# daigo0927/tf-raft

Measured on NVIDIA H100. Metric: frame-pairs/sec at 448×512 iters=12; final-flow max-abs vs ref, higher is better.
Workload: dtype f32

## Files before the change

include/raft_b200.h:

```cpp
#ifndef RAFT_B200_H_
#define RAFT_B200_H_

#include <stddef.h>
#include <stdint.h>

#ifdef __cplusplus
extern "C" {
#endif

#define RAFT_B200_ABI_VERSION 2
#define RAFT_MAX_LEVELS 8

typedef enum raft_status {
  RAFT_OK = 0,
  RAFT_ERR_BAD_ARG = -1,
  RAFT_ERR_BAD_SHAPE = -2,
  RAFT_ERR_WORKSPACE = -3,
  RAFT_ERR_NO_DEVICE = -4,
  RAFT_ERR_DRIVER = -5,
  RAFT_ERR_UNSUPPORTED = -6
} raft_status;

typedef enum raft_precision { RAFT_PREC_FP32 = 0, RAFT_PREC_F16X2 = 1 } raft_precision;

// ... 90 lines not shown
  RAFT_METRIC_LT1 = 1,
  RAFT_METRIC_LT3 = 2,
  RAFT_METRIC_LT5 = 3,
  RAFT_METRIC_OUTLIER = 4,
  RAFT_METRIC_COUNTS = 5
};

int raft_b200_flow_metrics_workspace_bytes(int B, int H, int W, size_t* bytes);

int raft_b200_flow_metrics(const float* pred, const float* gt, const float* valid, int B, int H, int W, int use_max_flow,
                           float max_flow, void* workspace, size_t workspace_bytes, long long* counts, double* sums,
                           void* stream);


typedef struct raft_conv {
  const float* kernel;
  const float* bias;
  int kh, kw, cin, cout;
} raft_conv;

typedef struct raft_basic_weights {
  raft_conv convc1, convc2, convf1, convf2, conv;
  raft_conv convz1, convr1, convq1, convz2, convr2, convq2;
  raft_conv fh_conv1, fh_conv2;
  raft_conv mask0, mask2;
} raft_basic_weights;

typedef struct raft_small_weights {
  raft_conv convc1, convf1, convf2, conv;
  raft_conv convz, convr, convq;
  raft_conv fh_conv1, fh_conv2;
} raft_small_weights;

int raft_b200_update_prepared_bytes(int variant, int corr_channels, int precision, size_t* bytes);
int raft_b200_update_prepare(int variant, const void* weights ,
                             void* prepared, size_t prepared_bytes, int precision, void* stream);

int raft_b200_update_workspace_bytes(int variant, int B, int h, int w, int precision, size_t* bytes);

int raft_b200_update_basic(const void* prepared, const float* net, const float* inp, const float* corr,
                           const float* flow, float* net_out, float* mask_or_null, float* delta_flow, int B,
                           int h, int w, void* workspace, size_t workspace_bytes, int precision, void* stream);

int raft_b200_update_small(const void* prepared, const float* net, const float* inp, const float* corr,
                           const float* flow, float* net_out, float* delta_flow, int B, int h, int w,
                           void* workspace, size_t workspace_bytes, int precision, void* stream);


typedef struct raft_norm {
  const float* gamma;
  const float* beta;
  const float* moving_mean;
  const float* moving_variance;
} raft_norm;

typedef struct raft_resblock {
  raft_conv conv1, conv2;
  raft_norm norm1, norm2;
  raft_conv downsample;
  raft_norm downsample_norm;
} raft_resblock;

typedef struct raft_encoder_weights {
  raft_conv conv1;
  raft_norm norm1;
  raft_resblock block[6];
  raft_conv conv2;
} raft_encoder_weights;

typedef enum raft_norm_type { RAFT_NORM_NONE = 0, RAFT_NORM_INSTANCE = 1, RAFT_NORM_BATCH = 2 } raft_norm_type;

int raft_b200_encoder_prepared_bytes(int variant, int out_dim, size_t* bytes);
int raft_b200_encoder_prepare(int variant, int norm_type, int out_dim, const raft_encoder_weights* weights,
                              void* prepared, size_t prepared_bytes, void* stream);
int raft_b200_encoder_workspace_bytes(int variant, int N, int H, int W, size_t* bytes);

int raft_b200_encoder_forward(int variant, int norm_type, int out_dim, const void* prepared, const float* images,
                              int N, int H, int W, int training, int image_norm, float* out, void* workspace,
                              size_t workspace_bytes, void* stream);

int raft_b200_context_split(const float* cnet, int npix, int hidden, int context, float* net, float* inp,
                            void* stream);

int raft_b200_conv2d(const float* x, const float* kernel, const float* bias, int B, int H, int W, int cin, int kh,
                     int kw, int cout, int act, float* out, int out_stride, int out_c0, void* stream);


int raft_b200_upsample_convex(const float* flow, const float* mask, int B, int h, int w, float* out, void* stream);

int raft_b200_upflow8(const float* flow, int B, int h, int w, float* out, void* stream);

int raft_b200_forward_loop(int variant, const void* prepared, const float* const pyr[], int levels, int radius,
                           float* net, const float* inp, float* coords1, float* const flow_up[], int iters,
                           int B, int h, int w, void* workspace, size_t workspace_bytes, int precision,
                           void* stream);

long long raft_b200_launch_count(void);
void raft_b200_launch_count_reset(void);
void raft_b200_profile_loop(int enable);
int raft_b200_profile_read(float* lookup_ms, float* update_ms, int* iterations);

#ifdef __cplusplus
}
#endif
#endif
```

tf_raft_b200/_lib.py:

```python
import ctypes
import os

import torch

_HERE = os.path.dirname(os.path.abspath(__file__))
LIB_PATH = os.environ.get('RAFT_B200_LIB') or os.path.join(_HERE, 'libraft_b200.so')

PREC_FP32 = 0
PREC_F16X2 = 1
VARIANT_BASIC = 0
VARIANT_SMALL = 1
MAX_LEVELS = 8

_PRECISIONS = {'fp32': PREC_FP32, 'f16x2': PREC_F16X2, PREC_FP32: PREC_FP32, PREC_F16X2: PREC_F16X2}


def resolve_precision(precision=None):
    if precision is None:
        precision = os.environ.get('RAFT_B200_PRECISION', 'f16x2')
    try:
        return _PRECISIONS[precision]
    except KeyError:
        raise ValueError(f'unknown precision {precision!r}; expected one of fp32, f16x2') from None


class RaftConv(ctypes.Structure):
    _fields_ = [('kernel', ctypes.c_void_p), ('bias', ctypes.c_void_p),
                ('kh', ctypes.c_int), ('kw', ctypes.c_int), ('cin', ctypes.c_int), ('cout', ctypes.c_int)]


class RaftNorm(ctypes.Structure):
    _fields_ = [('gamma', ctypes.c_void_p), ('beta', ctypes.c_void_p), ('moving_mean', ctypes.c_void_p),
                ('moving_variance', ctypes.c_void_p)]


class RaftResBlock(ctypes.Structure):
    _fields_ = [('conv1', RaftConv), ('conv2', RaftConv), ('norm1', RaftNorm), ('norm2', RaftNorm),
                ('downsample', RaftConv), ('downsample_norm', RaftNorm)]


class RaftEncoderWeights(ctypes.Structure):
    _fields_ = [('conv1', RaftConv), ('norm1', RaftNorm), ('block', RaftResBlock * 6), ('conv2', RaftConv)]


NORM_TYPES = {None: 0, 'instance': 1, 'batch': 2}

_vp, _i, _sz = ctypes.c_void_p, ctypes.c_int, ctypes.c_size_t
_SIGNATURES = {
    'raft_b200_strerror': (ctypes.c_char_p, [_i]),
    'raft_b200_abi_version': (_i, []),
    'raft_b200_device_ok': (_i, [_i]),
    'raft_b200_launch_count': (ctypes.c_longlong, []),
    'raft_b200_launch_count_reset': (None, []),
    'raft_b200_profile_loop': (None, [_i]),
    'raft_b200_profile_read': (_i, [ctypes.POINTER(ctypes.c_float), ctypes.POINTER(ctypes.c_float), ctypes.POINTER(_i)]),
    'raft_b200_corr_pyramid_sizes': (_i, [_i, _i, _i, _i, ctypes.POINTER(_sz)]),
    'raft_b200_corr_workspace_bytes': (_i, [_i, _i, _i, _i, _i, _i, ctypes.POINTER(_sz)]),
    'raft_b200_corr_pyramid_build': (_i, [_vp, _vp, _i, _i, _i, _i, _i, ctypes.POINTER(_vp), _vp, _sz, _i, _vp]),
    'raft_b200_corr_lookup': (_i, [ctypes.POINTER(_vp), _vp, _i, _i, _i, _i, _i, _vp, _i, _vp]),
    'raft_b200_corr_lookup_backward': (_i, [ctypes.POINTER(_vp), _vp, _vp, _i, _i, _i, _i, _i, _vp, ctypes.POINTER(_vp), _vp]),
    'raft_b200_sumsq': (_i, [_vp, _sz, _vp, _sz, _vp, _vp]),
    'raft_b200_adamw_step': (_i, [_vp, _vp, _vp, _vp, _sz, _vp, ctypes.c_float, ctypes.c_float, ctypes.c_float,
                                  ctypes.c_float, ctypes.c_float, ctypes.c_float, _vp]),
    'raft_b200_bilinear_sampler': (_i, [_vp, _vp, _i, _i, _i, _i, _vp, _vp]),
    'raft_b200_coords_grid': (_i, [_i, _i, _i, _vp, _vp]),
    'raft_b200_forward_interpolate': (_i, [_vp, _i, _i, _i, _vp, _vp]),
    'raft_b200_coords_init': (_i, [_vp, _i, _i, _i, _vp, _vp]),
    'raft_b200_fb_occlusion': (_i, [_vp, _vp, _i, _i, _i, ctypes.c_float, ctypes.c_float, _vp, _vp, _vp]),
    'raft_b200_augment_workspace_bytes': (_i, [_vp, _i, _i, ctypes.POINTER(_sz)]),
    'raft_b200_augment_dense': (_i, [_vp, _vp, _i, _vp, _sz, _vp]),
    'raft_b200_augment_sparse': (_i, [_vp, _vp, _i, _vp, _sz, _vp]),
    'raft_b200_flow_to_image': (_i, [_vp, _vp, _i, _i, _i, _i, _i, ctypes.c_float, _i, _vp, _i, _vp, _vp, _vp, _vp]),
    'raft_b200_png16_flow_decode': (_i, [_vp, _sz, _vp, _vp, _i, _vp, _vp]),
    'raft_b200_flow_metrics_workspace_bytes': (_i, [_i, _i, _i, ctypes.POINTER(_sz)]),
    'raft_b200_flow_metrics': (_i, [_vp, _vp, _vp, _i, _i, _i, _i, ctypes.c_float, _vp, _sz, _vp, _vp, _vp]),
    'raft_b200_update_prepared_bytes':(_i, [_i, _i, _i, ctypes.POINTER(_sz)]),
    'raft_b200_update_prepare': (_i, [_i, _vp, _vp, _sz, _i, _vp]),
    'raft_b200_update_workspace_bytes': (_i, [_i, _i, _i, _i, _i, ctypes.POINTER(_sz)]),
    'raft_b200_update_basic': (_i, [_vp, _vp, _vp, _vp, _vp, _vp, _vp, _vp, _i, _i, _i, _vp, _sz, _i, _vp]),
    'raft_b200_update_small': (_i, [_vp, _vp, _vp, _vp, _vp, _vp, _vp, _i, _i, _i, _vp, _sz, _i, _vp]),
    'raft_b200_upsample_convex': (_i, [_vp, _vp, _i, _i, _i, _vp, _vp]),
    'raft_b200_upflow8': (_i, [_vp, _i, _i, _i, _vp, _vp]),
    'raft_b200_encoder_prepared_bytes': (_i, [_i, _i, ctypes.POINTER(_sz)]),
    'raft_b200_encoder_prepare': (_i, [_i, _i, _i, _vp, _vp, _sz, _vp]),
    'raft_b200_encoder_workspace_bytes': (_i, [_i, _i, _i, _i, ctypes.POINTER(_sz)]),
    'raft_b200_encoder_forward': (_i, [_i, _i, _i, _vp, _vp, _i, _i, _i, _i, _i, _vp, _vp, _sz, _vp]),
    'raft_b200_context_split': (_i, [_vp, _i, _i, _i, _vp, _vp, _vp]),
    'raft_b200_conv2d': (_i, [_vp, _vp, _vp, _i, _i, _i, _i, _i, _i, _i, _i, _vp, _i, _i, _vp]),
    'raft_b200_forward_loop': (_i, [_i, _vp, ctypes.POINTER(_vp), _i, _i, _vp, _vp, _vp, ctypes.POINTER(_vp), _i,
                                    _i, _i, _i, _vp, _sz, _i, _vp]),
}
EXPORTED_SYMBOLS = tuple(_SIGNATURES)

_lib = None


def lib():
    global _lib
    if _lib is None:
        if not os.path.exists(LIB_PATH):
            raise ImportError(
                f'{LIB_PATH} is missing: the sm_90a CUDA library has not been built. '
                'Run `python -c "import __graft_entry__ as g; g.build()"` (or `python -m tf_raft_b200.build`) '
                'from the repository root. There is no CPU / PyTorch fallback for the RAFT hot path.')
        handle = ctypes.CDLL(LIB_PATH)
        for name, (res, args) in _SIGNATURES.items():
            fn = getattr(handle, name)
            fn.restype = res
            fn.argtypes = args
        if handle.raft_b200_abi_version() != 2:
            raise ImportError('libraft_b200.so ABI version mismatch; rebuild it')
        _lib = handle
    return _lib


def strerror(status):
    return lib().raft_b200_strerror(status).decode()


def check(status, what=''):
    if status != 0:
        raise RuntimeError(f'raft_b200 {what} failed: [{status}] {strerror(status)}')


def ptr(t):
    return ctypes.c_void_p(None if t is None else t.data_ptr())


def ptr_array(tensors):
    return (ctypes.c_void_p * len(tensors))(*[None if t is None else t.data_ptr() for t in tensors])


def stream():
    return ctypes.c_void_p(torch.cuda.current_stream().cuda_stream)


def require_cuda(*tensors):
    for t in tensors:
        if t is None:
            continue
        if not t.is_cuda:
            raise RuntimeError('tf_raft_b200 runs on CUDA tensors only (sm_90a); got a CPU tensor. '
                               'There is no CPU fallback for this path.')
        if t.dtype != torch.float32 or not t.is_contiguous():
            raise RuntimeError('expected contiguous float32 tensors')


def f32c(t):
    if not t.is_cuda:
        raise RuntimeError('tf_raft_b200 runs on CUDA tensors only (sm_90a); got a CPU tensor. '
                           'There is no CPU fallback for this path.')
    return t.to(torch.float32).contiguous()


def workspace(nbytes, device):
    return torch.empty(max(int(nbytes), 16), dtype=torch.uint8, device=device)


def launch_count():
    return int(lib().raft_b200_launch_count())


def launch_count_reset():
    lib().raft_b200_launch_count_reset()
```

tf_raft_b200/csrc/api.cu:

```cuda
#include <float.h>
#include <limits.h>
#include <stdlib.h>

#include <algorithm>

#include "augment.cuh"
#include "corr_tc.cuh"
#include "dataset.cuh"
#include "encoder.cuh"
#include "flow_viz.cuh"
#include "train.cuh"
#include "video.cuh"

namespace raft {
thread_local long long g_launches = 0;

static int check_dims(int B, int h, int w) { return (B > 0 && h > 0 && w > 0) ? 0 : RAFT_ERR_BAD_SHAPE; }
static int check_variant(int v) { return (v == RAFT_VARIANT_BASIC || v == RAFT_VARIANT_SMALL) ? 0 : RAFT_ERR_BAD_ARG; }
static int check_precision(int p) { return (p == RAFT_PREC_FP32 || p == RAFT_PREC_F16X2) ? 0 : RAFT_ERR_BAD_ARG; }

struct LoopProfile {
  bool on = false;
  int n = 0;
  cudaEvent_t ev[64][3];
// ... 31 lines not shown
  W.total = off;
  return W;
}

static int corr_build_fp32(const float* f1, const float* f2, int B, int h, int w, int C, int levels, float* const pyr[],
                           cudaStream_t st) {
  const int N = h * w;
  dim3 grid((unsigned)ceil_div(N, 64), (unsigned)ceil_div(N, 64), (unsigned)B);
  RAFT_TRY(launch(corr_fp32_kernel, grid, 256, 0, st, f1, f2, pyr[0], N, C, sqrtf((float)C)));
  int lh = h, lw = w;
  for (int l = 1; l < levels; ++l) {
    const size_t M = (size_t)B * N;
    const size_t total = M * (lh / 2) * (lw / 2);
    RAFT_TRY(launch(avgpool2x2_kernel, grid_for(total), 256, 0, st, pyr[l - 1], pyr[l], M, lh, lw, 1));
    lh /= 2;
    lw /= 2;
  }
  return 0;
}

static int corr_build_tc(const float* f1, const float* f2, int B, int h, int w, int C, int levels, float* const pyr[],
                         void* ws, cudaStream_t st) {
  if (C % kChunkK != 0) return RAFT_ERR_BAD_SHAPE;
  CorrWs W = corr_ws_layout(ws, B, h, w, C, levels, RAFT_PREC_F16X2);
  const int N = h * w;
  const size_t npix = (size_t)B * N;
  if (levels <= 4) {
    CorrPrepParams q;
    memset(&q, 0, sizeof(q));
    q.f1 = f1; q.f2 = f2; q.f1_hi = W.f1_hi; q.f1_lo = W.f1_lo;
    for (int l = 0; l < levels; ++l) { q.f2_hi[l] = W.f2_hi[l]; q.f2_lo[l] = W.f2_lo[l]; }
    q.B = B; q.h = h; q.w = w; q.C = C; q.levels = levels;
    q.patches_x = ceil_div(w, 8); q.patches_y = ceil_div(h, 8);
    q.npatch = B * q.patches_x * q.patches_y;
    const int split_blocks = (int)std::min<size_t>((npix * C / 4 + 127) / 128, (size_t)kNumSMs * 8);
    RAFT_TRY(launch(corr_prep_kernel, q.npatch + split_blocks, 128, 0, st, q));
  } else {
    RAFT_TRY(launch(split_plane_kernel, grid_for(npix * C), 256, 0, st, f1, C, 0, C, C, W.f1_hi, W.f1_lo, C, 0, npix, 1.0f));
    int lh = h, lw = w;
    const float* src = f2;
    for (int l = 0; l < levels; ++l) {
      if (l > 0) {
        const size_t total = (size_t)B * (lh / 2) * (lw / 2) * C;
        RAFT_TRY(launch(avgpool2x2_kernel, grid_for(total), 256, 0, st, src, W.f2_lvl[l], (size_t)B, lh, lw, C));
        src = W.f2_lvl[l];
        lh /= 2;
        lw /= 2;
      }
      const size_t np2 = (size_t)B * lh * lw;
      RAFT_TRY(launch(split_plane_kernel, grid_for(np2 * C), 256, 0, st, src, C, 0, C, C, W.f2_hi[l], W.f2_lo[l], C, 0, np2,
                      1.0f));
    }
  }

  CorrTcParams p;
  memset(&p, 0, sizeof(p));
  RAFT_TRY(make_tmap_act2(&p.a_map, W.f1_hi, W.f1_lo, B, 1, N, C, 128, 1));
  p.levels = levels; p.B = B; p.N = N; p.chunks = C / kChunkK;
  p.mtiles_img = ceil_div(N, kTileM);
  const int mtiles = B * p.mtiles_img;
  int lh = h, lw = w;
  for (int l = 0; l < levels; ++l) {
    const int N2 = lh * lw;
    const int ntn = ceil_div(N2, kCorrBn);
    const int bn = round_up(ceil_div(N2, ntn), 16);
    RAFT_TRY(make_tmap_wgt2(&p.b_map[l], W.f2_hi[l], W.f2_lo[l], B, N2, C, bn));
    p.out[l] = pyr[l];
    p.n2[l] = N2; p.bn[l] = bn;
    p.tile0[l + 1] = p.tile0[l] + mtiles * ntn;
    lh /= 2;
    lw /= 2;
  }
  p.corr_div = sqrtf((float)C);
  {
    int e = 0;
    const float m = frexpf(p.corr_div, &e);
    p.corr_mul = (m == 0.5f && p.corr_div * p.corr_div == (float)C) ? 1.0f / p.corr_div : 0.0f;
  }
  unsigned grid = 0;
  RAFT_TRY(persistent_grid<corr_tc_kernel>(kCorrSmemBytes, p.tile0[levels], &grid));
  return launch(corr_tc_kernel, grid, kTcThreads, kCorrSmemBytes, st, p);
}

static int update_begin(const UpdateCtx& c, const float* h, const float* inp) {
  const Workspace& W = c.W;
  const VariantDims d = variant_dims(c.variant);
  const size_t npix = (size_t)c.B * c.h * c.w;
  if (c.precision == RAFT_PREC_F16X2) {
    RAFT_CUDA_TRY(cudaMemsetAsync(W.f16_begin, 0, W.f16_bytes, c.stream));
    RAFT_TRY(launch(split_plane_kernel, grid_for(npix * d.ctx), 256, 0, c.stream, inp, d.ctx, 0, d.ctx, d.ctx, W.x_hi, W.x_lo,
                    d.s_x, 0, npix, 1.0f));
    return launch(split_plane_kernel, grid_for(npix * d.hid), 256, 0, c.stream, h, d.hid, 0, d.hid, d.hid, W.h_hi, W.h_lo,
                  d.s_h, 0, npix, 1.0f);
  }
  RAFT_CUDA_TRY(cudaMemsetAsync(W.x, 0, npix * d.c_x * sizeof(float), c.stream));
  return launch(copy_channels_kernel, grid_for(npix * d.ctx), 256, 0, c.stream, inp, d.ctx, 0, W.x, d.c_x, 0, d.ctx, npix);
}

static int make_ctx(UpdateCtx& c, int variant, const void* prepared, int B, int h, int w, void* ws, size_t ws_bytes,
                    int precision, void* stream) {
  RAFT_TRY(check_variant(variant));
  RAFT_TRY(check_precision(precision));
  if (!prepared || !ws) return RAFT_ERR_BAD_ARG;
  RAFT_TRY(check_dims(B, h, w));
  c.variant = variant; c.precision = precision; c.B = B; c.h = h; c.w = w;
  c.prepared = reinterpret_cast<const uint8_t*>(prepared);
  c.PL = prepared_layout(variant, precision);
  c.W = workspace_layout(ws, variant, B, h, w, precision);
  if (c.W.total > ws_bytes) return RAFT_ERR_WORKSPACE;
  c.stream = reinterpret_cast<cudaStream_t>(stream);
  c.plan = nullptr;
  c.fim_ready = false;
  return 0;
}

static bool mega_enabled() {
  static const int v = [] { const char* e = getenv("RAFT_B200_MEGA"); return e ? atoi(e) : 1; }();
  return v != 0;
}
static int update_block_tc(UpdateCtx& c, float* h, float* delta, float* mask, float* adv_coords) {
  MegaPlan plan;
  c.plan = mega_enabled() ? &plan : nullptr;
  const int st = update_core_tc(c, h, delta, mask, adv_coords);
  c.plan = nullptr;
  RAFT_TRY(st);
  if (!mega_enabled()) return 0;
  return mega_launch(plan, c.W.mega_flags, c.W.mega_flag_words, true, c.stream);
}

static int update_once(int variant, const void* prepared, const float* net, const float* inp, const float* corr,
                       const float* flow, float* net_out, float* mask, float* delta, int B, int h, int w, void* ws,
                       size_t ws_bytes, int precision, void* stream) {
  if (!net || !inp || !corr || !flow || !net_out || !delta) return RAFT_ERR_BAD_ARG;
  UpdateCtx c;
  RAFT_TRY(make_ctx(c, variant, prepared, B, h, w, ws, ws_bytes, precision, stream));
  const VariantDims d = variant_dims(variant);
  const size_t npix = (size_t)B * h * w;
  if (net_out != net)
    RAFT_CUDA_TRY(cudaMemcpyAsync(net_out, net, npix * d.hid * sizeof(float), cudaMemcpyDeviceToDevice, c.stream));
  RAFT_CUDA_TRY(cudaMemcpyAsync(c.W.flow, flow, npix * 2 * sizeof(float), cudaMemcpyDeviceToDevice, c.stream));
  RAFT_TRY(update_begin(c, net_out, inp));
  if (precision == RAFT_PREC_F16X2) {
    RAFT_TRY(launch(split_plane_kernel, grid_for(npix * d.s_corr), 256, 0, c.stream, corr, d.corr_ch, 0, d.corr_ch, d.s_corr,
                    c.W.corr_hi, c.W.corr_lo, d.s_corr, 0, npix, 1.0f));
    return update_block_tc(c, net_out, delta, mask, nullptr);
  }
  RAFT_CUDA_TRY(cudaMemcpyAsync(c.W.corr, corr, npix * d.corr_ch * sizeof(float), cudaMemcpyDeviceToDevice, c.stream));
  return update_core_fp32(c, net_out, delta, mask);
}

static int lookup_launch(const float* const pyr[], const float* coords, int B, int h, int w, int levels, int radius,
                         float* out, int out_stride, __half* out_hi, __half* out_lo, int h_stride, int h_pad,
                         cudaStream_t st, const float* im_flow = nullptr, __half* im_hi = nullptr, __half* im_lo = nullptr) {
  LookupParams p;
  memset(&p, 0, sizeof(p));
  int lh = h, lw = w;
  for (int l = 0; l < levels; ++l) {
    if (lh < 1 || lw < 1) return RAFT_ERR_BAD_SHAPE;
    p.pyr[l] = pyr[l];
    p.lh[l] = lh;
    p.lw[l] = lw;
    lh /= 2;
    lw /= 2;
  }
  p.coords = coords;
  p.out = out; p.out_stride = out_stride;
// ... 371 lines not shown
int raft_b200_update_workspace_bytes(int variant, int B, int h, int w, int precision, size_t* bytes) {
  if (!bytes) return RAFT_ERR_BAD_ARG;
  RAFT_TRY(check_variant(variant));
  RAFT_TRY(check_precision(precision));
  RAFT_TRY(check_dims(B, h, w));
  *bytes = workspace_layout(nullptr, variant, B, h, w, precision).total;
  return RAFT_OK;
}

int raft_b200_update_basic(const void* prepared, const float* net, const float* inp, const float* corr,
                           const float* flow, float* net_out, float* mask_or_null, float* delta_flow, int B, int h,
                           int w, void* workspace, size_t workspace_bytes, int precision, void* stream) {
  return update_once(RAFT_VARIANT_BASIC, prepared, net, inp, corr, flow, net_out, mask_or_null, delta_flow, B, h, w,
                     workspace, workspace_bytes, precision, stream);
}

int raft_b200_update_small(const void* prepared, const float* net, const float* inp, const float* corr,
                           const float* flow, float* net_out, float* delta_flow, int B, int h, int w, void* workspace,
                           size_t workspace_bytes, int precision, void* stream) {
  return update_once(RAFT_VARIANT_SMALL, prepared, net, inp, corr, flow, net_out, nullptr, delta_flow, B, h, w,
                     workspace, workspace_bytes, precision, stream);
}

int raft_b200_upsample_convex(const float* flow, const float* mask, int B, int h, int w, float* out, void* stream) {
  if (!flow || !mask || !out) return RAFT_ERR_BAD_ARG;
  RAFT_TRY(check_dims(B, h, w));
  const size_t npix = (size_t)B * h * w;
  return launch(upsample_convex_kernel, grid_for(npix, 4, kNumSMs * 32), 256, 0, reinterpret_cast<cudaStream_t>(stream), flow,
                mask, B, h, w, out);
}

int raft_b200_upflow8(const float* flow, int B, int h, int w, float* out, void* stream) {
  if (!flow || !out) return RAFT_ERR_BAD_ARG;
  RAFT_TRY(check_dims(B, h, w));
  return launch(upflow8_kernel, grid_for((size_t)B * h * w * 64), 256, 0, reinterpret_cast<cudaStream_t>(stream), flow, B, h,
                w, out);
}

int raft_b200_encoder_prepared_bytes(int variant, int out_dim, size_t* bytes) {
  if (!bytes) return RAFT_ERR_BAD_ARG;
  RAFT_TRY(check_variant(variant));
  if (out_dim < 32 || out_dim > 256 || out_dim % 32) return RAFT_ERR_BAD_SHAPE;
  *bytes = enc_layout(variant, out_dim).total;
  return RAFT_OK;
}

int raft_b200_encoder_prepare(int variant, int norm_type, int out_dim, const raft_encoder_weights* weights,
                              void* prepared, size_t prepared_bytes, void* stream) {
  if (!weights || !prepared) return RAFT_ERR_BAD_ARG;
  RAFT_TRY(check_variant(variant));
  if (norm_type < 0 || norm_type > 2) return RAFT_ERR_BAD_ARG;
  if (out_dim < 32 || out_dim > 256 || out_dim % 32) return RAFT_ERR_BAD_SHAPE;
  return encoder_prepare(variant, norm_type, out_dim, weights, prepared, prepared_bytes, reinterpret_cast<cudaStream_t>(stream));
}

int raft_b200_encoder_workspace_bytes(int variant, int N, int H, int W, size_t* bytes) {
  if (!bytes) return RAFT_ERR_BAD_ARG;
  RAFT_TRY(check_variant(variant));
  RAFT_TRY(check_dims(N, H, W));
  *bytes = enc_ws_layout(nullptr, variant, N, H, W).total;
  return RAFT_OK;
}

int raft_b200_encoder_forward(int variant, int norm_type, int out_dim, const void* prepared, const float* images,
                              int N, int H, int W, int training, int image_norm, float* out, void* workspace,
                              size_t workspace_bytes, void* stream) {
  if (!prepared || !images || !out || !workspace) return RAFT_ERR_BAD_ARG;
  RAFT_TRY(check_variant(variant));
  if (norm_type < 0 || norm_type > 2) return RAFT_ERR_BAD_ARG;
  RAFT_TRY(check_dims(N, H, W));
  if (out_dim < 32 || out_dim > 256 || out_dim % 32 || H < 8 || W < 8) return RAFT_ERR_BAD_SHAPE;
  return encoder_forward(variant, norm_type, out_dim, prepared, images, N, H, W, training, image_norm, out, workspace, workspace_bytes,
                         reinterpret_cast<cudaStream_t>(stream));
}

int raft_b200_context_split(const float* cnet, int npix, int hidden, int context, float* net, float* inp,
                            void* stream) {
  if (!cnet || !net || !inp) return RAFT_ERR_BAD_ARG;
  if (npix < 1 || hidden < 1 || context < 1) return RAFT_ERR_BAD_SHAPE;
  return launch(context_split_kernel, grid_for((size_t)npix * (hidden + context)), 256, 0, reinterpret_cast<cudaStream_t>(stream),
                cnet, (size_t)npix, hidden, context, net, inp);
}

int raft_b200_conv2d(const float* x, const float* kernel, const float* bias, int B, int H, int W, int cin, int kh,
                     int kw, int cout, int act, float* out, int out_stride, int out_c0, void* stream) {
  if (!x || !kernel || !out) return RAFT_ERR_BAD_ARG;
  RAFT_TRY(check_dims(B, H, W));
  if (cin < 1 || cout < 1 || kh < 1 || kw < 1 || !(kh & 1) || !(kw & 1) || act < 0 || act > 3) return RAFT_ERR_BAD_SHAPE;
  if (out_stride < out_c0 + cout) return RAFT_ERR_BAD_SHAPE;
  SimtConvParams p;
  memset(&p, 0, sizeof(p));
  p.src[0] = x; p.src_stride[0] = cin; p.src_c0[0] = 0; p.src_n[0] = cin; p.nsrc = 1;
  p.w = kernel; p.bias = bias;
  p.kh = kh; p.kw = kw; p.cin = cin; p.cout = cout;
  p.B = B; p.H = H; p.W = W;
  p.out = out; p.out_stride = out_stride; p.out_c0 = out_c0;
  p.act = act; p.out_scale = 1.0f;
  dim3 grid((unsigned)ceil_div(B * H * W, 64), (unsigned)ceil_div(cout, 64));
  return launch(conv_simt_kernel, grid, 256, 0, reinterpret_cast<cudaStream_t>(stream), p);
}

int raft_b200_forward_loop(int variant, const void* prepared, const float* const pyr[], int levels, int radius,
                           float* net, const float* inp, float* coords1, float* const flow_up[], int iters, int B,
                           int h, int w, void* workspace, size_t workspace_bytes, int precision, void* stream) {
  if (!pyr || !net || !inp || !coords1 || !flow_up || iters < 0) return RAFT_ERR_BAD_ARG;
  if (levels < 1 || levels > RAFT_MAX_LEVELS || radius < 0) return RAFT_ERR_BAD_ARG;
  UpdateCtx c;
  RAFT_TRY(make_ctx(c, variant, prepared, B, h, w, workspace, workspace_bytes, precision, stream));
  const VariantDims d = variant_dims(variant);
  const int side = 2 * radius + 1;
  if (levels * side * side != d.corr_ch) return RAFT_ERR_BAD_SHAPE;
  const size_t npix = (size_t)B * h * w;
  const Workspace& W = c.W;
  RAFT_TRY(update_begin(c, net, inp));
  RAFT_TRY(launch(flow_advance_kernel, grid_for(npix), 256, 0, c.stream, coords1, nullptr, W.flow, B, h, w));
  const bool prof = g_prof.on && iters <= 64;
  if (prof && !g_prof.created) {
    for (int i = 0; i < 64; ++i)
      for (int k = 0; k < 3; ++k) RAFT_CUDA_TRY(cudaEventCreate(&g_prof.ev[i][k]));
    g_prof.created = true;
  }
  if (prof) g_prof.n = iters;
  for (int i = 0; i < iters; ++i) {
    float* mask = (variant == RAFT_VARIANT_BASIC && flow_up[i]) ? W.mask : nullptr;
    if (precision == RAFT_PREC_F16X2) {
      if (prof) RAFT_CUDA_TRY(cudaEventRecord(g_prof.ev[i][0], c.stream));
      RAFT_TRY(lookup_launch(pyr, coords1, B, h, w, levels, radius, nullptr, 0, W.corr_hi, W.corr_lo, d.s_corr, d.s_corr,
                             c.stream, W.flow, W.fim_hi, W.fim_lo));
      if (prof) RAFT_CUDA_TRY(cudaEventRecord(g_prof.ev[i][1], c.stream));
      c.fim_ready = true;
      RAFT_TRY(update_block_tc(c, net, W.delta, mask, coords1));
      c.fim_ready = false;
      if (prof) RAFT_CUDA_TRY(cudaEventRecord(g_prof.ev[i][2], c.stream));
    } else {
      RAFT_TRY(lookup_launch(pyr, coords1, B, h, w, levels, radius, W.corr, d.corr_ch, nullptr, nullptr, 0, 0, c.stream));
      RAFT_TRY(update_core_fp32(c, net, W.delta, mask));
      RAFT_TRY(launch(flow_advance_kernel, grid_for(npix), 256, 0, c.stream, coords1, W.delta, W.flow, B, h, w));
    }
    if (flow_up[i]) {
      if (variant == RAFT_VARIANT_BASIC)
        RAFT_TRY(raft_b200_upsample_convex(W.flow, W.mask, B, h, w, flow_up[i], stream));
      else
        RAFT_TRY(raft_b200_upflow8(W.flow, B, h, w, flow_up[i], stream));
    }
  }
  return raft_launch_status();
}

}
```

tf_raft_b200/csrc/encoder.cuh:

```cuda
#pragma once
#include <algorithm>

#include "lookup.cuh"
#include "update.cuh"

namespace raft {

enum { NORM_NONE = 0, NORM_INSTANCE = 1, NORM_BATCH = 2 };

struct EncSpec { int c0; int c[3]; int s[3]; };
inline EncSpec enc_spec(int variant) {
  if (variant == RAFT_VARIANT_BASIC) return {64, {64, 96, 128}, {1, 2, 2}};
  return {32, {32, 64, 96}, {1, 2, 2}};
}
inline int pad64(int c) { return round_up(c, 64); }

struct EncNormSlot { size_t gamma, beta, fscale, fshift; int C; };
struct EncLayout {
  TcWeightSlot conv1;
  EncNormSlot norm1;
  TcWeightSlot bc1[6], bc2[6], bds[6];
  EncNormSlot bn1[6], bn2[6], bnd[6];
  int has_ds[6], bc[6], bstride[6];
  TcWeightSlot conv2;
// ... 99 lines not shown
  const EncLayout L = enc_layout(variant, out_dim);
  if (L.total > bytes) return RAFT_ERR_WORKSPACE;
  const EncSpec S = enc_spec(variant);
  uint8_t* base = reinterpret_cast<uint8_t*>(prepared);
  RAFT_CUDA_TRY(cudaMemsetAsync(base, 0, L.total, st));
  RAFT_TRY(enc_pack_conv(w->conv1, 7, 7, 3, S.c0, L.conv1, true, base, st));
  RAFT_TRY(enc_pack_norm(w->norm1, L.norm1, norm_type, base, st));
  int cin = S.c0;
  for (int k = 0; k < 6; ++k) {
    const int c = L.bc[k];
    RAFT_TRY(enc_pack_conv(w->block[k].conv1, 3, 3, cin, c, L.bc1[k], false, base, st));
    RAFT_TRY(enc_pack_conv(w->block[k].conv2, 3, 3, c, c, L.bc2[k], false, base, st));
    RAFT_TRY(enc_pack_norm(w->block[k].norm1, L.bn1[k], norm_type, base, st));
    RAFT_TRY(enc_pack_norm(w->block[k].norm2, L.bn2[k], norm_type, base, st));
    if (L.has_ds[k]) {
      RAFT_TRY(enc_pack_conv(w->block[k].downsample, 1, 1, cin, c, L.bds[k], false, base, st));
      RAFT_TRY(enc_pack_norm(w->block[k].downsample_norm, L.bnd[k], norm_type, base, st));
    }
    cin = c;
  }
  RAFT_TRY(enc_pack_conv(w->conv2, 1, 1, cin, out_dim, L.conv2, false, base, st));
  return raft_launch_status();
}

struct EncCtx {
  const uint8_t* prep; EncLayout L; EncWs W; cudaStream_t st;
  int N, norm_type, stats;
  int per_image;
};

inline int enc_norm_apply(const EncCtx& c, const EncNormSlot& ns, const float* y, size_t npix, int P, int relu,
                          const float* skip32, const __half* skip_hi, const __half* skip_lo, float* out32, __half* hi,
                          __half* lo) {
  const int C = ns.C, G = c.per_image ? c.N : 1;
  const int Pg = c.per_image ? P : (int)npix;
  const float* gamma = reinterpret_cast<const float*>(c.prep + ns.gamma);
  const float* beta = reinterpret_cast<const float*>(c.prep + ns.beta);
  RAFT_TRY(launch(norm_stats_kernel, dim3((unsigned)G, kNormSplit), 256, 0, c.st, y, Pg, C, kNormSplit, c.W.part));
  RAFT_TRY(launch(norm_final_kernel, ceil_div(G * C * 32, 256), 256, 0, c.st, c.W.part, G, C, kNormSplit, gamma, 1e-3f,
                  c.W.mean, c.W.mult));
  return launch(norm_apply_kernel, grid_for(npix * (pad64(C) / 8)), 256, 0, c.st, y, npix, P, C, c.per_image, c.W.mean,
                c.W.mult, beta, relu, skip32, skip_hi, skip_lo, out32, hi, lo, pad64(C));
}

inline int enc_conv_tc(const EncCtx& c, const TcWeightSlot& cs, int cout, const EncNormSlot* ns, const __half* ahi,
                       const __half* alo, int Hin, int Win, int Hout, int Wout, int stride, int relu, const float* skip,
                       float* out32, __half* ohi, __half* olo) {
  TcConvParams p;
  memset(&p, 0, sizeof(p));
  int tw, th;
  tc_pick_tile(Wout, Hout, &tw, &th);
  if (tw * stride > 256) tw = 128 / stride, th = 128 / tw;
  const int nsplit = tc_n_split(cs.cout_pad);
  if (!nsplit) return RAFT_ERR_BAD_SHAPE;
  RAFT_TRY(make_tmap_act2(&p.a_map[0], ahi, alo, c.N, Hin, Win, cs.cin_pad, tw, th, stride));
  RAFT_TRY(tc_use_weights(p, c.prep, cs, cs.cout_pad / nsplit));
  p.nseg = 1; p.seg_chunks[0] = cs.cin_pad / kChunkK; p.seg_c0[0] = 0;
  p.stride = stride;
  if (stride == 1) { p.ph = (cs.kh - 1) / 2; p.pw = (cs.kw - 1) / 2; }
  else {
    const int tot_h = (Hout - 1) * stride + cs.kh - Hin, tot_w = (Wout - 1) * stride + cs.kw - Win;
    p.ph = (tot_h > 0 ? tot_h : 0) / 2; p.pw = (tot_w > 0 ? tot_w : 0) / 2;
  }
  p.B = c.N; p.H = Hout; p.W = Wout; p.TH = th; p.TW = tw;
  p.n_total = cout;
  p.mode = EPI_LINEAR; p.out_scale = 1.0f;
  p.out_f32 = out32; p.f32_stride = cout; p.f32_c0 = 0;
  p.out_hi = ohi; p.out_lo = olo; p.h_stride = pad64(cout); p.h_c0 = 0;
  if (ns && !c.stats && c.norm_type == NORM_BATCH) {
    p.post_scale = reinterpret_cast<const float*>(c.prep + ns->fscale);
    p.post_shift = reinterpret_cast<const float*>(c.prep + ns->fshift);
  }
  const bool fused = !(ns && c.stats);
  if (fused) {
    p.act = relu ? ACT_RELU : ACT_NONE;
    p.residual = skip; p.res_stride = cout; p.res_c0 = 0;
  } else {
    p.act = ACT_NONE; p.out_hi = nullptr; p.out_lo = nullptr;
  }
  p.group_chunks = 5;
  return tc_launch(p, nsplit, c.st);
}

inline int encoder_forward(int variant, int norm_type, int out_dim, const void* prepared, const float* images, int N,
                           int H, int W, int training, int image_norm, float* out, void* ws, size_t ws_bytes, cudaStream_t st) {
  EncCtx c;
  c.prep = reinterpret_cast<const uint8_t*>(prepared);
  c.L = enc_layout(variant, out_dim);
  c.W = enc_ws_layout(ws, variant, N, H, W);
  if (c.W.total > ws_bytes) return RAFT_ERR_WORKSPACE;
  c.st = st; c.N = N; c.norm_type = norm_type;
  c.stats = (norm_type == NORM_INSTANCE) || (norm_type == NORM_BATCH && training);
  c.per_image = norm_type == NORM_INSTANCE;
  const EncSpec S = enc_spec(variant);
  const EncLayout& L = c.L;
  const EncWs& E = c.W;

  int h = (H + 1) / 2, w = (W + 1) / 2;
  {
    const size_t npix = (size_t)N * h * w;
    const int tot_h = (h - 1) * 2 + 7 - H, tot_w = (w - 1) * 2 + 7 - W;
    const float* src = images;
    if (image_norm) {
      const size_t nimg = (size_t)N * H * W * 3;
      RAFT_TRY(launch(image_norm_kernel, grid_for(nimg), 256, 0, st, images, E.O32, nimg));
      src = E.O32;
    }
    RAFT_TRY(launch(stem_im2col_kernel, grid_for(npix * 24), 256, 0, st, src, N, H, W, h, w, (tot_h > 0 ? tot_h : 0) / 2,
                    (tot_w > 0 ? tot_w : 0) / 2, 0, E.Ih, E.Il));
    if (!c.stats && pad64(S.c0) != S.c0) {
      RAFT_CUDA_TRY(cudaMemsetAsync(E.Xh, 0, npix * pad64(S.c0) * 2, st));
      RAFT_CUDA_TRY(cudaMemsetAsync(E.Xl, 0, npix * pad64(S.c0) * 2, st));
    }
    RAFT_TRY(enc_conv_tc(c, L.conv1, S.c0, &L.norm1, E.Ih, E.Il, h, w, h, w, 1, 1, nullptr, c.stats ? E.Y32 : E.X32, E.Xh, E.Xl));
    if (c.stats) RAFT_TRY(enc_norm_apply(c, L.norm1, E.Y32, npix, h * w, 1, nullptr, nullptr, nullptr, nullptr, E.Xh, E.Xl));
  }

  float *X32 = E.X32, *O32 = E.O32;
  __half *Xh = E.Xh, *Xl = E.Xl, *Oh = E.Oh, *Ol = E.Ol;
  for (int k = 0; k < 6; ++k) {
    const int st2 = L.bstride[k], cc = L.bc[k];
    const int ho = (h + st2 - 1) / st2, wo = (w + st2 - 1) / st2;
    const size_t npo = (size_t)N * ho * wo;
    const bool zero_pad_out = pad64(cc) != cc;
    if (!c.stats && zero_pad_out) {
      RAFT_CUDA_TRY(cudaMemsetAsync(E.Fh, 0, npo * pad64(cc) * 2, st));
      RAFT_CUDA_TRY(cudaMemsetAsync(E.Fl, 0, npo * pad64(cc) * 2, st));
      RAFT_CUDA_TRY(cudaMemsetAsync(Oh, 0, npo * pad64(cc) * 2, st));
      RAFT_CUDA_TRY(cudaMemsetAsync(Ol, 0, npo * pad64(cc) * 2, st));
    }
    RAFT_TRY(enc_conv_tc(c, L.bc1[k], cc, &L.bn1[k], Xh, Xl, h, w, ho, wo, st2, 1, nullptr, c.stats ? E.Y32 : nullptr, E.Fh, E.Fl));
    if (c.stats) RAFT_TRY(enc_norm_apply(c, L.bn1[k], E.Y32, npo, ho * wo, 1, nullptr, nullptr, nullptr, nullptr, E.Fh, E.Fl));
    const float* skip = X32;
    if (L.has_ds[k]) {
      RAFT_TRY(enc_conv_tc(c, L.bds[k], cc, &L.bnd[k], Xh, Xl, h, w, ho, wo, st2, 0, nullptr, c.stats ? E.Y32 : E.D32, nullptr, nullptr));
      if (c.stats) RAFT_TRY(enc_norm_apply(c, L.bnd[k], E.Y32, npo, ho * wo, 0, nullptr, nullptr, nullptr, E.D32, nullptr, nullptr));
      skip = E.D32;
    }
    RAFT_TRY(enc_conv_tc(c, L.bc2[k], cc, &L.bn2[k], E.Fh, E.Fl, ho, wo, ho, wo, 1, 1, skip, c.stats ? E.Y32 : O32, Oh, Ol));
    if (c.stats) {
      if (L.has_ds[k]) RAFT_TRY(enc_norm_apply(c, L.bn2[k], E.Y32, npo, ho * wo, 1, E.D32, nullptr, nullptr, nullptr, Oh, Ol));
      else RAFT_TRY(enc_norm_apply(c, L.bn2[k], E.Y32, npo, ho * wo, 1, nullptr, Xh, Xl, nullptr, Oh, Ol));
    }
    float* t32 = X32; X32 = O32; O32 = t32;
    __half* th_ = Xh; Xh = Oh; Oh = th_;
    __half* tl_ = Xl; Xl = Ol; Ol = tl_;
    h = ho; w = wo;
  }
  RAFT_TRY(enc_conv_tc(c, L.conv2, out_dim, nullptr, Xh, Xl, h, w, h, w, 1, 0, nullptr, out, nullptr, nullptr));
  return raft_launch_status();
}

}
```

tf_raft_b200/model.py:

```python
from collections import OrderedDict

import torch

from . import _lib
from .layers.corr import CorrBlock, coords_grid, coords_init, fb_occlusion, forward_interpolate, upflow8
from .layers.extractor import BasicEncoder, SmallEncoder
from .layers.update import BasicUpdateBlock, SmallUpdateBlock
from .losses import end_point_error, sequence_loss


class RAFT:
    _variant = _lib.VARIANT_BASIC

    def __init__(self, drop_rate=0, iters=12, iters_pred=24, *, precision=None, device='cuda', seed=None,
                 use_graph=False, encoder_backend=None, **kwargs):
        self.hidden_dim = 128
        self.context_dim = 128
        self.corr_levels = 4
        self.corr_radius = 4
        self.drop_rate = drop_rate
        self.iters = iters
        self.iters_pred = iters_pred
        self.precision = _lib.resolve_precision(precision)
        self.device = torch.device(device)
        self.use_graph = use_graph
        self.encoder_backend = encoder_backend
        self._build_layers(seed)
        self._graphs = {}
        self.flow_metrics = None
        self.optimizer = None
        self._trainer = None
        self._params_stale = False

    def _encoder_backend(self):
        return self.encoder_backend or ('native' if self.precision == _lib.PREC_F16X2 else 'torch')

    def _build_layers(self, seed):
        s = 0 if seed is None else seed
        self.fnet = BasicEncoder(output_dim=256, norm_type='instance', drop_rate=self.drop_rate, device=self.device,
                                 seed=s, backend=self._encoder_backend())
        self.cnet = BasicEncoder(output_dim=self.hidden_dim + self.context_dim, norm_type='batch',
                                 drop_rate=self.drop_rate, device=self.device, seed=s + 1, backend=self._encoder_backend())
        self.update_block = BasicUpdateBlock(filters=self.hidden_dim, precision=self.precision, device=self.device,
                                             seed=s + 2)

    def load_params(self, params):
        self.fnet.load_params(params, 'fnet.')
        self.cnet.load_params(params, 'cnet.')
        self.update_block.load_params(params, 'update_block.')
        self._graphs.clear()
        self._trainer = None
        self._params_stale = False

    def state_dict(self):
        self._sync_trained_params()
        out = OrderedDict()
        out.update(self.fnet.state_dict('fnet.'))
        out.update(self.cnet.state_dict('cnet.'))
        out.update(self.update_block.state_dict('update_block.'))
        return out

    def initialize_flow(self, image):
        bs, h, w, _ = image.shape
        return coords_grid(bs, h // 8, w // 8, self.device), coords_grid(bs, h // 8, w // 8, self.device)

    def upsample_flow(self, flow, mask):
        flow, mask = _lib.f32c(flow), _lib.f32c(mask)
        b, h, w, _ = flow.shape
        if tuple(mask.shape) != (b, h, w, 576):
            raise ValueError(f'mask: expected {(b, h, w, 576)}, got {tuple(mask.shape)}')
        out = torch.empty((b, 8 * h, 8 * w, 2), dtype=torch.float32, device=flow.device)
        with torch.cuda.device(flow.device):
            _lib.check(_lib.lib().raft_b200_upsample_convex(_lib.ptr(flow), _lib.ptr(mask), b, h, w, _lib.ptr(out),
                                                            _lib.stream()), 'upsample_convex')
        return out

    def _encode(self, image1, image2, training):
        fmap1, fmap2 = self.fnet([image1, image2], training=training, raw_image=True)
        net, inp = self._context(image1, training)
        return fmap1, fmap2, net, inp

    def _context(self, image1, training):
        cnet = self.cnet(image1, training=training, raw_image=True)
        b, h, w, _ = cnet.shape
        net = torch.empty((b, h, w, self.hidden_dim), dtype=torch.float32, device=cnet.device)
        inp = torch.empty((b, h, w, self.context_dim), dtype=torch.float32, device=cnet.device)
        with torch.cuda.device(cnet.device):
            _lib.check(_lib.lib().raft_b200_context_split(_lib.ptr(cnet), b * h * w, self.hidden_dim,
                                                          self.context_dim, _lib.ptr(net), _lib.ptr(inp),
                                                          _lib.stream()), 'context_split')
        return net, inp

    def _loop(self, corr_block, net, inp, coords1, flow_ups, b, h, w):
        ub = self.update_block
        ws = ub.workspace(b, h, w)
        with torch.cuda.device(self.device):
            _lib.check(_lib.lib().raft_b200_forward_loop(
                self._variant, _lib.ptr(ub.prepared()), _lib.ptr_array(corr_block.corr_pyramid), self.corr_levels,
                self.corr_radius, _lib.ptr(net), _lib.ptr(inp), _lib.ptr(coords1), _lib.ptr_array(flow_ups),
                len(flow_ups), b, h, w, _lib.ptr(ws), ws.numel(), self.precision, _lib.stream()), 'forward_loop')

    def __call__(self, inputs, training, *, last_only=False, flow_init=None):
        image1, image2 = inputs
        image1, image2 = _lib.f32c(image1), _lib.f32c(image2)
        if flow_init is not None:
            flow_init = self._check_flow_init(flow_init, image1)
        self._sync_trained_params()
        if self.use_graph and not training:
            key = (tuple(image1.shape), bool(last_only), flow_init is not None)
            return self._graph_run(key, lambda a, b, f: self._forward(a, b, False, last_only, f),
                                   (image1, image2, flow_init))
        return self._forward(image1, image2, training, last_only, flow_init)

    @staticmethod
    def _check_flow_init(flow_init, image):
        if not isinstance(flow_init, torch.Tensor):
            raise TypeError(f'flow_init must be a torch tensor, got {type(flow_init).__name__}')
        if flow_init.dtype != torch.float32:
            raise TypeError(f'flow_init must be float32, got {flow_init.dtype}')
        if flow_init.device != image.device:
            raise ValueError(f'flow_init is on {flow_init.device}, the images on {image.device}')
        bs, H, W, _ = image.shape
        want = (bs, H // 8, W // 8, 2)
        if tuple(flow_init.shape) != want:
            raise ValueError(f'flow_init: expected {want} for {H}x{W} images, got {tuple(flow_init.shape)}')
        return flow_init.contiguous()

    def _graph_run(self, key, fn, inputs):
        entry = self._graphs.get(key)
        if entry is None:
            statics = [None if t is None else t.clone() for t in inputs]
            side = torch.cuda.Stream(device=self.device)
            side.wait_stream(torch.cuda.current_stream(self.device))
            with torch.cuda.stream(side):
                for _ in range(2):
                    fn(*statics)
            torch.cuda.current_stream(self.device).wait_stream(side)
            torch.cuda.synchronize(self.device)
            graph = torch.cuda.CUDAGraph()
            with torch.cuda.graph(graph):
                outs = fn(*statics)
            keep = [list(m._ws.values()) for m in (self.fnet, self.cnet, self.update_block)]
            entry = (graph, statics, outs, self._last, keep)
            self._graphs[key] = entry
        graph, statics, outs, last, _keep = entry
        for s, t in zip(statics, inputs):
            if t is not None:
                s.copy_(t, non_blocking=True)
        graph.replay()
        self._last = last
        return outs

    @staticmethod
    def _check_size(H, W):
        if H % 8 or W % 8:
            raise ValueError(f'image height and width must be multiples of 8 (got {H}x{W}); the reference fails in '
                             'update.py:146 for other sizes -- crop-or-pad first (datasets/dataset.py:323-334)')

    def _forward(self, image1, image2, training, last_only, flow_init=None):
        bs, H, W, _ = image1.shape
        self._check_size(H, W)
        fmap1, fmap2, net, inp = self._encode(image1, image2, training)
        return self._iterate(fmap1, fmap2, net, inp, bs, H, W, training, last_only, flow_init)

    def _iterate(self, fmap1, fmap2, net, inp, bs, H, W, training, last_only, flow_init):
        h, w = H // 8, W // 8
        iters = self.iters if training else self.iters_pred
        corr_block = CorrBlock(fmap1, fmap2, num_levels=self.corr_levels, radius=self.corr_radius,
                               precision=self.precision)
        if flow_init is None:
            coords1 = coords_grid(bs, h, w, self.device)
        else:
            coords1 = coords_init(flow_init)
        preds = [torch.empty((bs, H, W, 2), dtype=torch.float32, device=self.device)
                 if (not last_only or i == iters - 1) else None for i in range(iters)]
        if iters:
            self._loop(corr_block, net, inp, coords1, preds, bs, h, w)
        self._last = dict(net=net, coords1=coords1, corr_block=corr_block)
        return [p for p in preds if p is not None] if last_only else preds

    def predict_bidirectional(self, inputs):
        image1, image2 = inputs
        image1, image2 = _lib.f32c(image1), _lib.f32c(image2)
        if image1.shape != image2.shape:
            raise ValueError(f'image1 {tuple(image1.shape)} and image2 {tuple(image2.shape)} differ in shape')
        if self.iters_pred < 1:
            raise ValueError('predict_bidirectional needs iters_pred >= 1')
        self._sync_trained_params()
        if self.use_graph:
            return self._graph_run(('bidirectional', tuple(image1.shape)), self._bidirectional, (image1, image2))
        return self._bidirectional(image1, image2)

    def _bidirectional(self, image1, image2):
        bs, H, W, _ = image1.shape
        self._check_size(H, W)
        images = torch.cat([image1, image2])
        fmap = self.fnet(images, training=False, raw_image=True)
        net, inp = self._context(images, False)
        return self._iterate_bidirectional(fmap, torch.cat([fmap[bs:], fmap[:bs]]), net, inp, bs, H, W, None)

    def _iterate_bidirectional(self, fmap1, fmap2, net, inp, bs, H, W, flow_init):
        flow = self._iterate(fmap1, fmap2, net, inp, 2 * bs, H, W, False, True, flow_init)[-1]
        flow_fw, flow_bw = flow[:bs], flow[bs:]
        return (flow_fw, flow_bw) + fb_occlusion(flow_fw, flow_bw)

    def predict_video(self, frames, *, warm_start=True, bidirectional=False):
        self._sync_trained_params()
        if self.iters_pred < 1:
            raise ValueError('predict_video needs iters_pred >= 1')
        shape = coords0 = frame_prev = fmap_prev = flow_init = ctx_prev = None
        for t, frame in enumerate(frames):
            frame = _lib.f32c(frame)
            if shape is None:
                shape = tuple(frame.shape)
                if len(shape) != 4 or shape[-1] != 3:
                    raise ValueError(f'frames must be (B, H, W, 3); got {shape}')
                bs, H, W, _ = shape
                self._check_size(H, W)
            elif tuple(frame.shape) != shape:
                raise ValueError(f'frame {t}: shape {tuple(frame.shape)} differs from the first frame {shape}')
            fmap = self.fnet(frame, training=False, raw_image=True)
            if bidirectional:
                ctx = self._context(frame, False)
            if frame_prev is not None:
                if bidirectional:
# ... 99 lines not shown
```

Before: 311.8.

## Run fnet and cnet encoders concurrently on side streams with shared stem im2col

Adds a fused encode_pair entry point that forks the caller stream into three streams. fnet on image2, fnet on image1 and cnet on image1 then run concurrently, and the image1 stem normalisation and im2col is computed once and shared by both image1 encoders. The goal is to fill the GPU during the small-batch encoder phase and drop one redundant stem pass. In exchange it adds per-device static streams and events, a larger workspace holding three encoder scratch areas, and stream-priority choices that may interact with CUDA graph capture.

```diff
diff --git a/include/raft_b200.h b/include/raft_b200.h
--- a/include/raft_b200.h
+++ b/include/raft_b200.h
@@ -196,6 +196,12 @@
 int raft_b200_context_split(const float* cnet, int npix, int hidden, int context, float* net, float* inp,
                             void* stream);
 
+int raft_b200_encode_pair_workspace_bytes(int variant, int N, int H, int W, int cnet_dim, size_t* bytes);
+int raft_b200_encode_pair(int variant, const void* fnet_prepared, int fnet_norm, int fnet_dim, const void* cnet_prepared,
+                          int cnet_norm, int hidden, int context, const float* image1, const float* image2, int N, int H,
+                          int W, float* fmap1, float* fmap2, float* net, float* inp, void* workspace, size_t workspace_bytes,
+                          void* stream);
+
 int raft_b200_conv2d(const float* x, const float* kernel, const float* bias, int B, int H, int W, int cin, int kh,
                      int kw, int cout, int act, float* out, int out_stride, int out_c0, void* stream);
 
diff --git a/tf_raft_b200/_lib.py b/tf_raft_b200/_lib.py
--- a/tf_raft_b200/_lib.py
+++ b/tf_raft_b200/_lib.py
@@ -86,6 +86,9 @@
     'raft_b200_encoder_workspace_bytes': (_i, [_i, _i, _i, _i, ctypes.POINTER(_sz)]),
     'raft_b200_encoder_forward': (_i, [_i, _i, _i, _vp, _vp, _i, _i, _i, _i, _i, _vp, _vp, _sz, _vp]),
     'raft_b200_context_split': (_i, [_vp, _i, _i, _i, _vp, _vp, _vp]),
+    'raft_b200_encode_pair_workspace_bytes': (_i, [_i, _i, _i, _i, _i, ctypes.POINTER(_sz)]),
+    'raft_b200_encode_pair': (_i, [_i, _vp, _i, _i, _vp, _i, _i, _i, _vp, _vp, _i, _i, _i, _vp, _vp, _vp, _vp, _vp, _sz,
+                                   _vp]),
     'raft_b200_conv2d': (_i, [_vp, _vp, _vp, _i, _i, _i, _i, _i, _i, _i, _i, _vp, _i, _i, _vp]),
     'raft_b200_forward_loop': (_i, [_i, _vp, ctypes.POINTER(_vp), _i, _i, _vp, _vp, _vp, ctypes.POINTER(_vp), _i,
                                     _i, _i, _i, _vp, _sz, _i, _vp]),
diff --git a/tf_raft_b200/csrc/api.cu b/tf_raft_b200/csrc/api.cu
--- a/tf_raft_b200/csrc/api.cu
+++ b/tf_raft_b200/csrc/api.cu
@@ -137,6 +137,49 @@
   return launch(corr_tc_kernel, grid, kTcThreads, kCorrSmemBytes, st, p);
 }
 
+struct PairWs {
+  void* enc[3];
+  size_t enc_bytes;
+  const __half *stem_hi, *stem_lo;
+  float* cnet_out;
+  size_t total;
+};
+static PairWs pair_ws_layout(void* base, int variant, int N, int H, int W, int cnet_dim) {
+  PairWs P;
+  memset(&P, 0, sizeof(P));
+  uint8_t* b8 = reinterpret_cast<uint8_t*>(base);
+  P.enc_bytes = align_up(enc_ws_layout(nullptr, variant, N, H, W).total, 1024);
+  for (int i = 0; i < 3; ++i) P.enc[i] = b8 + i * P.enc_bytes;
+  const EncWs E = enc_ws_layout(P.enc[0], variant, N, H, W);
+  P.stem_hi = E.Ih; P.stem_lo = E.Il;
+  P.cnet_out = reinterpret_cast<float*>(b8 + 3 * P.enc_bytes);
+  P.total = 3 * P.enc_bytes + (size_t)N * ceil_div(H, 8) * ceil_div(W, 8) * cnet_dim * sizeof(float);
+  return P;
+}
+
+struct PairStreams { cudaStream_t s[3]; cudaEvent_t fork, stem, a, b, c; bool ready; };
+static int pair_streams(cudaStream_t caller, PairStreams** out) {
+  static thread_local PairStreams tab[64];
+  int dev = 0;
+  RAFT_CUDA_TRY(cudaGetDevice(&dev));
+  if (dev < 0 || dev >= 64) return RAFT_ERR_UNSUPPORTED;
+  PairStreams& ps = tab[dev];
+  if (!ps.ready) {
+    cudaStreamCaptureStatus cs = cudaStreamCaptureStatusNone;
+    RAFT_CUDA_TRY(cudaStreamIsCapturing(caller, &cs));
+    if (cs != cudaStreamCaptureStatusNone) return RAFT_ERR_UNSUPPORTED;
+    int least = 0, greatest = 0;
+    RAFT_CUDA_TRY(cudaDeviceGetStreamPriorityRange(&least, &greatest));
+    for (int i = 0; i < 3; ++i)
+      RAFT_CUDA_TRY(cudaStreamCreateWithPriority(&ps.s[i], cudaStreamNonBlocking, i < 2 ? greatest : least));
+    for (cudaEvent_t* e : {&ps.fork, &ps.stem, &ps.a, &ps.b, &ps.c})
+      RAFT_CUDA_TRY(cudaEventCreateWithFlags(e, cudaEventDisableTiming));
+    ps.ready = true;
+  }
+  *out = &ps;
+  return RAFT_OK;
+}
+
 static int update_begin(const UpdateCtx& c, const float* h, const float* inp) {
   const Workspace& W = c.W;
   const VariantDims d = variant_dims(c.variant);
@@ -674,6 +717,57 @@
                 cnet, (size_t)npix, hidden, context, net, inp);
 }
 
+int raft_b200_encode_pair_workspace_bytes(int variant, int N, int H, int W, int cnet_dim, size_t* bytes) {
+  if (!bytes) return RAFT_ERR_BAD_ARG;
+  RAFT_TRY(check_variant(variant));
+  RAFT_TRY(check_dims(N, H, W));
+  if (cnet_dim < 1) return RAFT_ERR_BAD_SHAPE;
+  *bytes = pair_ws_layout(nullptr, variant, N, H, W, cnet_dim).total;
+  return RAFT_OK;
+}
+
+int raft_b200_encode_pair(int variant, const void* fnet_prepared, int fnet_norm, int fnet_dim, const void* cnet_prepared,
+                          int cnet_norm, int hidden, int context, const float* image1, const float* image2, int N, int H,
+                          int W, float* fmap1, float* fmap2, float* net, float* inp, void* workspace, size_t workspace_bytes,
+                          void* stream) {
+  if (!fnet_prepared || !cnet_prepared || !image1 || !image2 || !fmap1 || !fmap2 || !net || !inp || !workspace)
+    return RAFT_ERR_BAD_ARG;
+  RAFT_TRY(check_variant(variant));
+  if (fnet_norm < 0 || fnet_norm > 2 || cnet_norm < 0 || cnet_norm > 2) return RAFT_ERR_BAD_ARG;
+  RAFT_TRY(check_dims(N, H, W));
+  const int cnet_dim = hidden + context;
+  for (int d : {fnet_dim, cnet_dim})
+    if (d < 32 || d > 256 || d % 32) return RAFT_ERR_BAD_SHAPE;
+  if (hidden < 1 || context < 1 || H < 8 || W < 8) return RAFT_ERR_BAD_SHAPE;
+  const int h = ceil_div(H, 8), w = ceil_div(W, 8);
+  const PairWs P = pair_ws_layout(workspace, variant, N, H, W, cnet_dim);
+  if (P.total > workspace_bytes) return RAFT_ERR_WORKSPACE;
+  cudaStream_t st = reinterpret_cast<cudaStream_t>(stream);
+  PairStreams* ps = nullptr;
+  RAFT_TRY(pair_streams(st, &ps));
+  cudaStream_t sa = ps->s[0], sb = ps->s[1], sc = ps->s[2];
+  const size_t enc_bytes = P.enc_bytes;
+
+  RAFT_CUDA_TRY(cudaEventRecord(ps->fork, st));
+  for (cudaStream_t s : {sa, sb, sc}) RAFT_CUDA_TRY(cudaStreamWaitEvent(s, ps->fork, 0));
+  int status = encoder_stem_im2col(variant, image1, N, H, W, 1, P.enc[0], sa);
+  if (!status) status = (int)cudaEventRecord(ps->stem, sa);
+  if (!status) status = encoder_forward(variant, fnet_norm, fnet_dim, fnet_prepared, image2, N, H, W, 0, 1, fmap2, P.enc[1],
+                                        enc_bytes, sb);
+  if (!status) status = (int)cudaStreamWaitEvent(sc, ps->stem, 0);
+  if (!status) status = encoder_forward(variant, cnet_norm, cnet_dim, cnet_prepared, image1, N, H, W, 0, 1, P.cnet_out, P.enc[2],
+                                        enc_bytes, sc, P.stem_hi, P.stem_lo);
+  if (!status) status = launch(context_split_kernel, grid_for((size_t)N * h * w * cnet_dim), 256, 0, sc, P.cnet_out,
+                               (size_t)N * h * w, hidden, context, net, inp);
+  if (!status) status = encoder_forward(variant, fnet_norm, fnet_dim, fnet_prepared, image1, N, H, W, 0, 1, fmap1, P.enc[0],
+                                        enc_bytes, sa, P.stem_hi, P.stem_lo);
+  RAFT_CUDA_TRY(cudaEventRecord(ps->a, sa));
+  RAFT_CUDA_TRY(cudaEventRecord(ps->b, sb));
+  RAFT_CUDA_TRY(cudaEventRecord(ps->c, sc));
+  for (cudaEvent_t e : {ps->a, ps->b, ps->c}) RAFT_CUDA_TRY(cudaStreamWaitEvent(st, e, 0));
+  return status ? status : raft_launch_status();
+}
+
 int raft_b200_conv2d(const float* x, const float* kernel, const float* bias, int B, int H, int W, int cin, int kh,
                      int kw, int cout, int act, float* out, int out_stride, int out_c0, void* stream) {
   if (!x || !kernel || !out) return RAFT_ERR_BAD_ARG;
diff --git a/tf_raft_b200/csrc/encoder.cuh b/tf_raft_b200/csrc/encoder.cuh
--- a/tf_raft_b200/csrc/encoder.cuh
+++ b/tf_raft_b200/csrc/encoder.cuh
@@ -205,8 +205,25 @@
   return tc_launch(p, nsplit, c.st);
 }
 
+inline int encoder_stem_im2col(int variant, const float* images, int N, int H, int W, int image_norm, void* ws,
+                               cudaStream_t st) {
+  const EncWs E = enc_ws_layout(ws, variant, N, H, W);
+  const int h = (H + 1) / 2, w = (W + 1) / 2;
+  const size_t npix = (size_t)N * h * w;
+  const int tot_h = (h - 1) * 2 + 7 - H, tot_w = (w - 1) * 2 + 7 - W;
+  const float* src = images;
+  if (image_norm) {
+    const size_t nimg = (size_t)N * H * W * 3;
+    RAFT_TRY(launch(image_norm_kernel, grid_for(nimg), 256, 0, st, images, E.O32, nimg));
+    src = E.O32;
+  }
+  return launch(stem_im2col_kernel, grid_for(npix * 24), 256, 0, st, src, N, H, W, h, w, (tot_h > 0 ? tot_h : 0) / 2,
+                (tot_w > 0 ? tot_w : 0) / 2, 0, E.Ih, E.Il);
+}
+
 inline int encoder_forward(int variant, int norm_type, int out_dim, const void* prepared, const float* images, int N,
-                           int H, int W, int training, int image_norm, float* out, void* ws, size_t ws_bytes, cudaStream_t st) {
+                           int H, int W, int training, int image_norm, float* out, void* ws, size_t ws_bytes, cudaStream_t st,
+                           const __half* stem_hi = nullptr, const __half* stem_lo = nullptr) {
   EncCtx c;
   c.prep = reinterpret_cast<const uint8_t*>(prepared);
   c.L = enc_layout(variant, out_dim);
@@ -222,20 +239,15 @@
   int h = (H + 1) / 2, w = (W + 1) / 2;
   {
     const size_t npix = (size_t)N * h * w;
-    const int tot_h = (h - 1) * 2 + 7 - H, tot_w = (w - 1) * 2 + 7 - W;
-    const float* src = images;
-    if (image_norm) {
-      const size_t nimg = (size_t)N * H * W * 3;
-      RAFT_TRY(launch(image_norm_kernel, grid_for(nimg), 256, 0, st, images, E.O32, nimg));
-      src = E.O32;
-    }
-    RAFT_TRY(launch(stem_im2col_kernel, grid_for(npix * 24), 256, 0, st, src, N, H, W, h, w, (tot_h > 0 ? tot_h : 0) / 2,
-                    (tot_w > 0 ? tot_w : 0) / 2, 0, E.Ih, E.Il));
+    if (!stem_hi) {
+      RAFT_TRY(encoder_stem_im2col(variant, images, N, H, W, image_norm, ws, st));
+      stem_hi = E.Ih; stem_lo = E.Il;
+    }
     if (!c.stats && pad64(S.c0) != S.c0) {
       RAFT_CUDA_TRY(cudaMemsetAsync(E.Xh, 0, npix * pad64(S.c0) * 2, st));
       RAFT_CUDA_TRY(cudaMemsetAsync(E.Xl, 0, npix * pad64(S.c0) * 2, st));
     }
-    RAFT_TRY(enc_conv_tc(c, L.conv1, S.c0, &L.norm1, E.Ih, E.Il, h, w, h, w, 1, 1, nullptr, c.stats ? E.Y32 : E.X32, E.Xh, E.Xl));
+    RAFT_TRY(enc_conv_tc(c, L.conv1, S.c0, &L.norm1, stem_hi, stem_lo, h, w, h, w, 1, 1, nullptr, c.stats ? E.Y32 : E.X32, E.Xh, E.Xl));
     if (c.stats) RAFT_TRY(enc_norm_apply(c, L.norm1, E.Y32, npix, h * w, 1, nullptr, nullptr, nullptr, nullptr, E.Xh, E.Xl));
   }
 
diff --git a/tf_raft_b200/model.py b/tf_raft_b200/model.py
--- a/tf_raft_b200/model.py
+++ b/tf_raft_b200/model.py
@@ -1,3 +1,4 @@
+import ctypes
 from collections import OrderedDict
 
 import torch
@@ -27,6 +28,7 @@
         self.encoder_backend = encoder_backend
         self._build_layers(seed)
         self._graphs = {}
+        self._pair_ws = {}
         self.flow_metrics = None
         self.optimizer = None
         self._trainer = None
@@ -76,6 +78,8 @@
         return out
 
     def _encode(self, image1, image2, training):
+        if not training and self.fnet.backend == self.cnet.backend == 'native':
+            return self._encode_pair(image1, image2)
         fmap1, fmap2 = self.fnet([image1, image2], training=training, raw_image=True)
         net, inp = self._context(image1, training)
         return fmap1, fmap2, net, inp
@@ -90,6 +94,31 @@
                                                           self.context_dim, _lib.ptr(net), _lib.ptr(inp),
                                                           _lib.stream()), 'context_split')
         return net, inp
+
+    def _encode_pair(self, image1, image2):
+        bs, H, W, _ = image1.shape
+        h, w = -(-H // 8), -(-W // 8)
+        dev = image1.device
+        L = _lib.lib()
+        key = (bs, H, W)
+        if key not in self._pair_ws:
+            nbytes = ctypes.c_size_t()
+            _lib.check(L.raft_b200_encode_pair_workspace_bytes(self._variant, bs, H, W, self.hidden_dim + self.context_dim,
+                                                               ctypes.byref(nbytes)), 'encode_pair_workspace_bytes')
+            self._pair_ws = {key: _lib.workspace(nbytes.value, dev)}
+        ws = self._pair_ws[key]
+        fmap1 = torch.empty((bs, h, w, self.fnet.output_dim), dtype=torch.float32, device=dev)
+        fmap2 = torch.empty_like(fmap1)
+        net = torch.empty((bs, h, w, self.hidden_dim), dtype=torch.float32, device=dev)
+        inp = torch.empty((bs, h, w, self.context_dim), dtype=torch.float32, device=dev)
+        fnet, cnet = self.fnet, self.cnet
+        with torch.cuda.device(dev):
+            _lib.check(L.raft_b200_encode_pair(
+                self._variant, _lib.ptr(fnet.prepared()), _lib.NORM_TYPES[fnet.norm_type], fnet.output_dim,
+                _lib.ptr(cnet.prepared()), _lib.NORM_TYPES[cnet.norm_type], self.hidden_dim, self.context_dim,
+                _lib.ptr(image1), _lib.ptr(image2), bs, H, W, _lib.ptr(fmap1), _lib.ptr(fmap2), _lib.ptr(net), _lib.ptr(inp),
+                _lib.ptr(ws), ws.numel(), _lib.stream()), 'encode_pair')
+        return fmap1, fmap2, net, inp
 
     def _loop(self, corr_block, net, inp, coords1, flow_ups, b, h, w):
         ub = self.update_block
@@ -140,7 +169,7 @@
             graph = torch.cuda.CUDAGraph()
             with torch.cuda.graph(graph):
                 outs = fn(*statics)
-            keep = [list(m._ws.values()) for m in (self.fnet, self.cnet, self.update_block)]
+            keep = [list(m._ws.values()) for m in (self.fnet, self.cnet, self.update_block)] + [list(self._pair_ws.values())]
             entry = (graph, statics, outs, self._last, keep)
             self._graphs[key] = entry
         graph, statics, outs, last, _keep = entry
```

New measurement: 325.2, median of 6. +4.3%, better.
